# cxm12/TGSR

Measured on AMD Instinct MI355X. Metric: SR images/sec (32->256, batch 16 per GPU, one step in flight), higher is better.
Workload: dtype f32

## Files before the change

### include/tgsr_hip.h

```cpp
#ifndef TGSR_HIP_H
#define TGSR_HIP_H

#include <stdint.h>

#ifdef __cplusplus
extern "C" {
#endif

#define TGSR_OK 0
#define TGSR_EINVAL (-1)
#define TGSR_EUNSUPPORTED (-2)
#define TGSR_ELAUNCH (-3)

#define TGSR_EPI_AFFINE 0
#define TGSR_EPI_AFFINE_GLU 1

#define TGSR_ACT_NONE 0
#define TGSR_ACT_TANH_AXPY 1
#define TGSR_ACT_IDENT_AXPY 2

#define TGSR_ABI_VERSION 2
int tgsr_abi_version(void);
const char* tgsr_last_error(void);

// ... 40 lines not shown
                           float* out, int64_t out_bstride, int epilogue, void* stream);

int tgsr_pack_wino4_wide_weight(const float* w, float* upack, int Cout, int Cin, int glu, void* stream);
int tgsr_pack_wino4_wide_weight_dgrad(const float* w, float* upack, int Cout, int Cin, void* stream);
int tgsr_wino4_wide_stats_nslots(int B, int H, int W, int Cout);
int tgsr_wino4_wide_conv3x3_stats_fwd(const float* x, int64_t x_bstride, int B, int Cin, int H, int W, const float* upack,
                                      int Cout, float* out, int64_t out_bstride, float* stat_partial, void* stream);
int tgsr_wino4_wide_conv3x3_fwd(const float* x, int64_t x_bstride, int B, int Cin, int H, int W, const float* upack, int Cout,
                                const float* scale, const float* shift, const float* residual, int64_t res_bstride,
                                float* out, int64_t out_bstride, int epilogue, void* stream);

int tgsr_conv_to3_set_pipe(int on);

int tgsr_conv_to3_fwd(const float* x, int64_t x_bstride, int B, int Cin, int H, int W, const float* w, int K,
                      int act, const float* addend, float alpha, float* out, void* stream);

int tgsr_word_attention_fwd(const float* h, int64_t h_bstride, const float* words, const float* w_ctx,
                            const uint8_t* mask, int mask_mode, int B, int idf, int cdf, int T, int Q, float* src_ws,
                            float* c_code, int64_t c_bstride, float* attn, void* stream);

int tgsr_word_project_fwd(const float* words, const float* const* w_ctx, int nsets, int B, int idf, int cdf, int T,
                          float* src_out, void* stream);

int tgsr_bilstm_fwd(const int64_t* captions, int width, const int32_t* cap_lens, int B, int Tmax, const float* emb,
                    int ntoken, int ninput, const float* w_ih, const float* w_hh, const float* b_ih,
                    const float* b_hh, int H, float* gates_ws, float* words_emb, float* sent_emb, void* stream);

int tgsr_lstm_gate_table(const float* emb, int ntoken, int ninput, const float* w_ih, const float* b_ih,
                         const float* b_hh, int H, float* table, void* stream);
int tgsr_bilstm_table_fwd(const int64_t* captions, int width, const int32_t* cap_lens, int B, int Tmax,
// ... 271 lines not shown
```

### tgsr_amd/_lib.py

```python
import ctypes
import os
import subprocess

_HERE = os.path.dirname(os.path.abspath(__file__))
LIB_PATH = os.environ.get("TGSR_LIB_PATH") or os.path.join(_HERE, "lib", "libtgsr_hip.so")
ABI_VERSION = 2

OK, EINVAL, EUNSUPPORTED, ELAUNCH = 0, -1, -2, -3
EPI_AFFINE, EPI_AFFINE_GLU = 0, 1
ACT_NONE, ACT_TANH_AXPY, ACT_IDENT_AXPY = 0, 1, 2
DT_BF16, DT_F16 = 1, 2

_vp, _i, _i64, _f, _d = ctypes.c_void_p, ctypes.c_int, ctypes.c_int64, ctypes.c_float, ctypes.c_double

SIGNATURES = {
    "tgsr_abi_version": (_i, []),
    "tgsr_last_error": (ctypes.c_char_p, []),
    "tgsr_packed_weight_elems": (_i64, [_i, _i, _i]),
    "tgsr_pack_conv_weight": (_i, [_vp, _vp, _i, _i, _i, _vp]),
    "tgsr_pack_conv_weight_dgrad": (_i, [_vp, _vp, _i, _i, _i, _vp]),
    "tgsr_bn_fold": (_i, [_vp, _vp, _vp, _vp, _f, _vp, _vp, _i, _vp]),
    "tgsr_conv3x3_fwd": (_i, [_vp, _i64, _i, _i, _i, _i, _vp, _i, _vp, _vp, _vp, _i64, _vp, _i64, _i, _i, _vp]),
    "tgsr_packed_upconv_weight_elems": (_i64, [_i, _i]),
    "tgsr_pack_upconv_weight": (_i, [_vp, _vp, _i, _i, _vp]),
# ... 30 lines not shown
    "tgsr_damsm_words_bwd_ws_elems": (_i64, [_i, _i, _i]),
    "tgsr_damsm_words_bwd": (_i, [_vp, _vp, _vp, _vp, _i, _i, _i, _i, _f, _f, _vp, _vp, _vp, _vp]),
    "tgsr_func_attention_fwd": (_i, [_vp, _vp, _i, _i, _i, _i, _f, _vp, _vp, _vp]),
    "tgsr_conv1x1_fwd": (_i, [_vp, _i, _i, _i, _vp, _vp, _i, _vp, _vp]),
    "tgsr_linear_fwd": (_i, [_vp, _i, _i, _vp, _vp, _i, _vp, _vp]),
    "tgsr_rowdot_fwd": (_i, [_vp, _vp, _vp, _vp, _i, _i, _vp]),
    "tgsr_ca_net_fwd": (_i, [_vp, _vp, _vp, _vp, _i, _i, _i, _vp, _vp, _vp, _vp]),
    "tgsr_rowdot_bwd": (_i, [_vp, _vp, _vp, _vp, _vp, _i, _i, _vp]),
    "tgsr_bn_train_nsplit": (_i, [_i, _i, _i]),
    "tgsr_bn_train_fwd": (_i, [_vp, _i, _i, _i, _vp, _vp, _f, _f, _vp, _vp, _i, _vp, _i64, _vp, _vp, _vp, _vp, _vp, _vp,
                               _i64, _vp, _vp]),
    "tgsr_bn_train_bwd": (_i, [_vp, _vp, _i, _i, _i, _vp, _vp, _vp, _vp, _i, _vp, _vp, _vp, _vp, _vp, _vp]),
    "tgsr_dconv_set_split": (_i, [_i]),
    "tgsr_bn_set_fuse_small": (_i, [_i]),
    "tgsr_conv_to3_set_pipe": (_i, [_i]),
    "tgsr_conv4x4s2_split_form": (_i, [_i, _i, _i, _i, _i, _i]),
    "tgsr_conv3x3_gemm_split_form": (_i, [_i, _i, _i, _i, _i, _i]),
    "tgsr_conv4x4s2_ws_elems": (_i64, [_i, _i, _i, _i, _i, _i]),
    "tgsr_conv4x4s2_fwd": (_i, [_vp, _i, _i, _i, _i, _vp, _i, _i, _vp, _vp, _vp]),
    "tgsr_conv4x4s2_dgrad": (_i, [_vp, _i, _i, _i, _i, _vp, _i, _vp, _vp, _vp]),
    "tgsr_conv4x4s2_wgrad": (_i, [_vp, _vp, _i, _i, _i, _i, _i, _vp, _vp, _vp]),
    "tgsr_conv3x3_gemm_ws_elems": (_i64, [_i, _i, _i, _i, _i, _i]),
    "tgsr_conv3x3_gemm_fwd": (_i, [_vp, _i, _i, _i, _i, _vp, _i, _vp, _vp, _vp]),
    "tgsr_conv3x3_gemm_dgrad": (_i, [_vp, _i, _i, _i, _i, _vp, _i, _vp, _vp, _vp]),
    "tgsr_conv3x3_gemm_wgrad": (_i, [_vp, _vp, _i, _i, _i, _i, _i, _vp, _vp, _vp]),
    "tgsr_leaky_relu": (_i, [_vp, _vp, _vp, _i64, _vp]),
    "tgsr_glu": (_i, [_vp, _vp, _vp, _i64, _i64, _vp]),
    "tgsr_wino_stats_nslots": (_i, [_i, _i, _i, _i]),
    "tgsr_wino_conv3x3_stats_fwd": (_i, [_vp, _i64, _i, _i, _i, _i, _vp, _i, _vp, _i64, _vp, _vp]),
    "tgsr_wino4_stats_nslots": (_i, [_i, _i, _i, _i]),
# ... 135 lines not shown
```

### tgsr_amd/csrc/tgsr_conv_to3.hip

```cpp
#include "tgsr_common.h"

namespace tgsr {

typedef __attribute__((address_space(3))) void* lds_ptr3_t;
typedef const __attribute__((address_space(1))) void* glb_ptr1_t;

__device__ __attribute__((aligned(16))) float g_to3_zero[4] = {0.f, 0.f, 0.f, 0.f};

struct To3Args {
  const float* x;
  int64_t xbs;
  int B, Cin, H, W;
  const float* w;
  const float* addend;
  float alpha;
  float* out;
  int tiles_x, tiles_y;
};

__device__ __forceinline__ float fast_tanh(float v) {
  const float e = __expf(2.f * v);
  return 1.f - 2.f / (e + 1.f);
}

// ... 143 lines not shown
          if (xx + p < a.W) {
            float v = acc[co][p];
            if (ACT == TGSR_ACT_TANH_AXPY) {
              v = fast_tanh(v);
              if (addp) v += a.alpha * addp[o + p];
            }
            outp[o + p] = v;
          }
        }
      }
    }
  }
}


template <int K, int ACT, int TH, int KS>
__global__ __launch_bounds__(16 * TH * KS) void conv_to3_pipe_kernel(To3Args a) {
  constexpr int P = K / 2, CK = 2, TW = 64, NG = 16 * TH, NW = NG / 64, NT = 16 * TH * KS;
  constexpr int TR = TH + K - 1;
  constexpr int PITCH = 72;
  constexpr int STAGE = CK * TR * PITCH;
  constexpr int UK = ((STAGE + 255) / 256 + NW - 1) / NW;
  constexpr int BUF = UK * NW * 256, D = 3;
  constexpr int WPC = (3 * K * K + 3) & ~3;
  static_assert(NG % 64 == 0, "a channel group is a whole number of waves");
  static_assert((KS - 1) * 12 * NG <= KS * D * BUF, "reduction buffer fits the stage buffers");
  __shared__ __attribute__((aligned(16))) float smem_all[KS * D * BUF];
  extern __shared__ __attribute__((aligned(16))) float w_s[];

  const int grp = __builtin_amdgcn_readfirstlane(threadIdx.x / NG);
  const int tid = threadIdx.x - grp * NG, lane = tid & 63;
  const int wave = __builtin_amdgcn_readfirstlane(tid >> 6);
  float* smem = smem_all + grp * D * BUF;
  const int lq = (lane >> 2) & 7;
  const int txi = (lq >> 1) * 4 + (lane & 3), tyi = 4 * wave + 2 * (lane >> 5) + ((0x96 >> lq) & 1);
  int t = xcd_remap(blockIdx.x, gridDim.x);
  const int tx = t % a.tiles_x;
  t /= a.tiles_x;
  const int ty = t % a.tiles_y;
  const int b = t / a.tiles_y;
  const int y0 = ty * TH, x0 = tx * TW;
  const uint32_t HW = (uint32_t)a.H * (uint32_t)a.W;
  const float* xb = a.x + (int64_t)b * a.xbs;

  for (int o = threadIdx.x; o < a.Cin * 3 * K * K; o += NT) {
    const int c = o / (3 * K * K), r = o - c * (3 * K * K);
    const int co = r / (K * K), tp = r - co * (K * K);
    w_s[c * WPC + r] = a.w[((int64_t)co * a.Cin + c) * (K * K) + tp];
  }

  int off[UK];
// ... 13 lines not shown
    for (int k = 0; k < UK; ++k) {
      const int v = off[k];
      const int c = c0 + (v >> 28);
      const bool ok = v >= 0 && c < a.Cin;
      const float* g = ok ? xb + (uint64_t)(uint32_t)c * HW + (uint32_t)(v & 0x0fffffff) : g_to3_zero;
      const unsigned dst = lds0 + (unsigned)(bi * BUF + NW * k * 256) * 4u;
      asm volatile("s_mov_b32 m0, %1\n\ts_nop 0\n\tglobal_load_lds_dwordx4 %0, off" ::"v"(g), "s"(dst) : "memory");
    }
  };

  float acc[3][4];
#pragma unroll
  for (int co = 0; co < 3; ++co)
#pragma unroll
    for (int p = 0; p < 4; ++p) acc[co][p] = 0.f;

  const int nst = (a.Cin + CK - 1) / CK, per = (nst + KS - 1) / KS;
  const int s0 = grp * per, s1 = s0 + per < nst ? s0 + per : nst;
  if (s0 < s1) issue(0, s0 * CK);
  if (s0 + 1 < s1) issue(1, (s0 + 1) * CK);
  __syncthreads();

  int bi = 0;
  for (int i = 0; i < per; ++i) {
    const int st = s0 + i;
    if (st + 1 < s1) asm volatile("s_waitcnt vmcnt(%0)\n\ts_barrier" ::"n"(UK) : "memory");
    else asm volatile("s_waitcnt vmcnt(0)\n\ts_barrier" ::: "memory");
    if (st + 2 < s1) issue(bi >= 1 ? bi - 1 : 2, (st + 2) * CK);
    const float* cur = smem + bi * BUF;
    const int c0 = st * CK;
// ... 34 lines not shown
#pragma unroll
      for (int co = 0; co < 3; ++co)
#pragma unroll
        for (int p = 0; p < 4; ++p) red[((grp - 1) * 12 + co * 4 + p) * NG + tid] = acc[co][p];
    }
    __syncthreads();
    if (grp > 0) return;
#pragma unroll
    for (int g = 1; g < KS; ++g)
#pragma unroll
      for (int co = 0; co < 3; ++co)
#pragma unroll
        for (int p = 0; p < 4; ++p) acc[co][p] += red[((g - 1) * 12 + co * 4 + p) * NG + tid];
  }

  const int y = y0 + tyi, xx = x0 + 4 * txi;
  float* __restrict__ outp = a.out;
  const float* __restrict__ addp = a.addend;
  if (y < a.H && xx < a.W) {
#pragma unroll
    for (int co = 0; co < 3; ++co) {
      const int64_t o = ((int64_t)b * 3 + co) * HW + (int64_t)y * a.W + xx;
      float4 ad = make_float4(0.f, 0.f, 0.f, 0.f);
      if (ACT == TGSR_ACT_TANH_AXPY && addp) ad = *reinterpret_cast<const float4*>(addp + o);
      const float adv[4] = {ad.x, ad.y, ad.z, ad.w};
      float r[4];
#pragma unroll
      for (int p = 0; p < 4; ++p) r[p] = ACT == TGSR_ACT_TANH_AXPY ? fast_tanh(acc[co][p]) + a.alpha * adv[p] : acc[co][p];
      *reinterpret_cast<float4*>(outp + o) = make_float4(r[0], r[1], r[2], r[3]);
    }
  }
}

template <int K, int ACT, int CH, int TRO>
__global__ __launch_bounds__(256) void conv_to3_mfma_kernel(To3Args a) {
  constexpr int RPW = TRO / 4;
  constexpr int NJ = CH / 4;
  constexpr int P = K / 2, ROWS = TRO + K - 1, PITCH = 80;
  constexpr int CS = (ROWS * PITCH) % 64 == 0 ? ROWS * PITCH + 16 : (ROWS * PITCH + 63) / 64 * 64 + 16 - ((ROWS * PITCH) % 64 <= 16 ? 64 : 0);
  static_assert(CS % 64 == 16 && CS >= ROWS * PITCH && CS % 4 == 0, "channel stride");
  constexpr int VP = 84;
  constexpr int SM = CH * CS > 4 * 16 * VP ? CH * CS : 4 * 16 * VP;
  __shared__ __attribute__((aligned(16))) float x_s[SM];
  const int tid = threadIdx.x, lane = tid & 63, wave = tid >> 6, col = lane & 15, kq = lane >> 4;
// ... 94 lines not shown
        if (a.addend) v += a.alpha * a.addend[o];
      }
      a.out[o] = v;
    }
    asm volatile("s_waitcnt lgkmcnt(0)" ::: "memory");
    __builtin_amdgcn_wave_barrier();
  }
}

static int g_to3_pipe = [] {
  const char* e = getenv("TGSR_TO3_PIPE");
  return (e && e[0] == '0') ? 0 : 1;
}();
static bool to3_pipe() { return g_to3_pipe != 0; }

template <int K, int ACT, int TH, int KS>
static int launch_to3_th(To3Args a, hipStream_t s) {
  a.tiles_x = (a.W + 63) / 64;
  a.tiles_y = (a.H + TH - 1) / TH;
  const dim3 grid((unsigned)(a.B * a.tiles_x * a.tiles_y));
  const bool vec4 = (a.W % 4 == 0) && (a.xbs % 4 == 0) && ((reinterpret_cast<uintptr_t>(a.x) & 15) == 0) &&
                    ((reinterpret_cast<uintptr_t>(a.out) & 15) == 0) &&
                    (!a.addend || (reinterpret_cast<uintptr_t>(a.addend) & 15) == 0);
  constexpr int WPC = (3 * K * K + 3) & ~3;
  const size_t wbytes = (size_t)a.Cin * WPC * sizeof(float);
  if (vec4 && wbytes <= 16 * 1024 && to3_pipe())
    hipLaunchKernelGGL((conv_to3_pipe_kernel<K, ACT, TH, KS>), grid, dim3(16 * TH * KS), wbytes, s, a);
  else if (vec4)
    hipLaunchKernelGGL((conv_to3_kernel<K, ACT, true, TH, KS>), grid, dim3(16 * TH * KS), 0, s, a);
  else
    hipLaunchKernelGGL((conv_to3_kernel<K, ACT, false, TH, KS>), grid, dim3(16 * TH * KS), 0, s, a);
  return note_launch(hipGetLastError(), "conv_to3_kernel");
}

template <int K, int ACT>
static int launch_to3(To3Args a, hipStream_t s) {
  auto tiles = [&](int th) { return (int64_t)a.B * ((a.W + 63) / 64) * ((a.H + th - 1) / th); };
  if (K == 5 && a.Cin % 16 == 0 && a.W % 64 == 0 && a.H % 8 == 0 && tiles(8) >= 512 && a.xbs % 4 == 0 &&
      (reinterpret_cast<uintptr_t>(a.x) & 15) == 0) {
    a.tiles_x = a.W / 64;
    a.tiles_y = a.H / 8;
    hipLaunchKernelGGL((conv_to3_mfma_kernel<K, ACT, 8, 8>), dim3((unsigned)(a.B * a.tiles_x * a.tiles_y)), dim3(256), 0, s, a);
    return note_launch(hipGetLastError(), "conv_to3_mfma_kernel");
  }
  if (tiles(16) >= 512) return launch_to3_th<K, ACT, 16, 1>(a, s);
  if (tiles(8) >= 512) return launch_to3_th<K, ACT, 8, 2>(a, s);
  return launch_to3_th<K, ACT, 4, 4>(a, s);
}

}

using namespace tgsr;

extern "C" int tgsr_conv_to3_set_pipe(int on) {
  const int was = g_to3_pipe;
  g_to3_pipe = on ? 1 : 0;
  return was;
}

extern "C" int tgsr_conv_to3_fwd(const float* x, int64_t x_bstride, int B, int Cin, int H, int W, const float* w,
                                 int K, int act, const float* addend, float alpha, float* out, void* stream) {
  if (!x || !w || !out || B < 1 || Cin < 1 || H < 1 || W < 1) return TGSR_EINVAL;
  if (K != 3 && K != 5) return TGSR_EUNSUPPORTED;
  if (act != TGSR_ACT_NONE && act != TGSR_ACT_TANH_AXPY) return TGSR_EINVAL;
  if (act == TGSR_ACT_NONE && addend) return TGSR_EINVAL;
  if ((int64_t)H * W >= (1 << 28) || (int64_t)Cin * H * W >= (1ll << 32)) return TGSR_EUNSUPPORTED;
  To3Args a;
  a.x = x; a.xbs = x_bstride; a.B = B; a.Cin = Cin; a.H = H; a.W = W; a.w = w;
  a.addend = addend; a.alpha = alpha; a.out = out; a.tiles_x = a.tiles_y = 0;
  hipStream_t s = as_stream(stream);
  if (K == 3) return act == TGSR_ACT_NONE ? launch_to3<3, TGSR_ACT_NONE>(a, s) : launch_to3<3, TGSR_ACT_TANH_AXPY>(a, s);
  return act == TGSR_ACT_NONE ? launch_to3<5, TGSR_ACT_NONE>(a, s) : launch_to3<5, TGSR_ACT_TANH_AXPY>(a, s);
}
```

### tgsr_amd/custom_ops.py

```python
from typing import Optional

import torch

from . import lp, ops

_lib = torch.library.Library("tgsr", "DEF")
_T = torch.Tensor


def _refuse_cpu(name):
    def kernel(*args, **kwargs):
        raise ops.TgsrError("torch.ops.tgsr.%s got CPU tensors: tgsr_amd ops run only on HIP tensors; there is no CPU fallback" % name)
    return kernel


def _define(schema, fn, fake=None):
    name = schema.split("(")[0]
    _lib.define(schema)
    _lib.impl(name, fn, "CUDA")
    _lib.impl(name, _refuse_cpu(name), "CPU")
    if fake is not None:
        torch.library.register_fake("tgsr::" + name, fake, lib=_lib)
    return getattr(torch.ops.tgsr, name).default

# ... 388 lines not shown
                    (words.new_empty(len(ws), words.shape[0], ws[0].shape[0], 32), words.new_empty(words.shape[0], ncf),
                     words.new_empty(words.shape[0], ncf),
                     words.new_empty(words.shape[0], words.shape[2], dtype=torch.uint8)))
text_tail_lp = _define("text_tail_lp(Tensor words, Tensor[] w_ctxs, Tensor sent_emb, Tensor ca_w, Tensor ca_b, int ncf, "
                       "Tensor captions, bool bf16) -> (Tensor, Tensor, Tensor, Tensor, Tensor)",
                       lambda words, ws, sent, cw, cb, ncf, cap, bf16:
                       ops.text_tail(words, list(ws), sent, cw, cb, ncf, cap,
                                     lp_dtype=torch.bfloat16 if bf16 else torch.float16),
                       lambda words, ws, sent, cw, cb, ncf, cap, bf16:
                       (words.new_empty(len(ws), words.shape[0], ws[0].shape[0], 32), words.new_empty(words.shape[0], ncf),
                        words.new_empty(words.shape[0], ncf),
                        words.new_empty(words.shape[0], words.shape[2], dtype=torch.uint8),
                        words.new_empty(len(ws) * words.shape[0] * 4096 + 4 * words.shape[0], dtype=torch.uint8)))
axpy_images = _define("axpy_images(Tensor[] ts, Tensor[] ss, float alpha) -> Tensor[]",
                      lambda ts, ss, alpha: ops.axpy_images(list(ts), list(ss), alpha), lambda ts, ss, alpha: [torch.empty_like(t) for t in ts])
gconv_pack = _define("gconv_pack(Tensor w, Tensor? scale, bool dgrad) -> Tensor", lambda w, sc, dg: ops.gconv_pack(w, sc, dg),
                     lambda w, sc, dg: w.new_empty((w.shape[1], w.shape[0] * w.shape[2] * w.shape[3]) if dg else
                                                   (w.shape[0], w.shape[1] * w.shape[2] * w.shape[3])))
gconv = _define("gconv(bool dgrad, Tensor A, Tensor S, int s_coff, int s_ch, Tensor(a!) out, int o_coff, int kh, int kw, int stride, "
                "int padh, int padw, Tensor? bias, bool relu, bool accumulate, Tensor(b!)? ws, Tensor? mask) -> ()",
                lambda dg, A, S, sc, sch, out, oc, kh, kw, st, ph, pw, bias, relu, acc, ws, mask:
                ops.gconv(dg, A, S, sc, sch, out, oc, kh, kw, st, ph, pw, bias, relu, acc, ws, mask), lambda *a: None)
gconv_stats = _define("gconv_stats(Tensor A, Tensor S, int s_coff, int s_ch, Tensor(a!) out, int o_coff, int kh, int kw, int stride, "
                      "int padh, int padw, Tensor(b!)? ws, Tensor(c!) stat_partial) -> ()",
                      lambda A, S, sc, sch, out, oc, kh, kw, st, ph, pw, ws, part:
                      (ops.gconv_stats(A, S, sc, sch, out, oc, kh, kw, st, ph, pw, ws, part), None)[1], lambda *a: None)
bn_train_relu_slice_from_stats = _define(
    "bn_train_relu_slice_from_stats(Tensor(a!) y, int coff, Tensor gamma, Tensor beta, float eps, float momentum, "
    "Tensor(b!)? running_mean, Tensor(c!)? running_var, Tensor(d!)? num_batches_tracked, Tensor stat_partial, int slot_px, "
    "Tensor(e!) stats) -> ()",
# ... 162 lines not shown
```

### tgsr_amd/model.py

```python
import torch
import torch.nn as nn
import torch.nn.functional as F
from torch.autograd import Variable

from . import custom_ops as C
from . import ops
from .miscc.config import cfg
from .util import (CA_NET, CNN_ENCODER, D_GET_LOGITS, GET_IMAGE_G, GET_IMAGE_G_noAct, GLU, INIT_STAGE_GImgup, NEXT_STAGE_G,
                   RNN_ENCODER, ResBlock, Block3x3_leakRelu, Block3x3_relu, _ConvBnGlu, _ResidualNoSum, conv1x1, conv3x3,
                   conv5x5, downBlock, encode_image_by_16times, upBlock)

__all__ = ["G_SR_NET_low", "G_SR_NET_low_stage1", "NetG_highweight", "RNN_ENCODER", "CNN_ENCODER", "CA_NET",
           "INIT_STAGE_GImgup", "NEXT_STAGE_G", "GET_IMAGE_G", "GET_IMAGE_G_noAct", "ResBlock", "GLU", "upBlock",
           "Block3x3_relu", "conv1x1", "conv3x3", "conv5x5", "Variable", "cfg", "torch", "nn", "F",
           "D_NET64", "D_NET128", "D_NET256", "D_GET_LOGITS", "downBlock", "Block3x3_leakRelu"]


class G_SR_NET_low_stage1(nn.Module):

    def __init__(self, *args, **kwargs):
        super(G_SR_NET_low_stage1, self).__init__()
        raise NotImplementedError("G_SR_NET_low_stage1 is dead code in the reference (stage1=False, "
                                  "trainer_objective.py:56); tgsr_amd builds G_SR_NET_low")

# ... 4 lines not shown
        super(G_SR_NET_low, self).__init__()
        ngf = cfg.GAN.GF_DIM
        nef = cfg.TEXT.EMBEDDING_DIM
        ncf = cfg.GAN.CONDITION_DIM
        self.ca_net = CA_NET()
        self.h_net1 = INIT_STAGE_GImgup(ngf, ncf, nef)
        self.h_net2 = NEXT_STAGE_G(ngf, nef, ncf)
        self.h_net3 = NEXT_STAGE_G(ngf, nef, ncf)
        self.img_net1 = GET_IMAGE_G_noAct(ngf)
        self.img_net2 = GET_IMAGE_G_noAct(ngf)
        self.img_net3 = GET_IMAGE_G_noAct(ngf)

    def attention_modules(self):
        return [self.h_net1.att, self.h_net2.att, self.h_net3.att]

    def forward(self, LR, sent_emb, word_embs, mask, outmiddle=False, ca=None, proj=None):
        fake_imgs, att_maps = [], []
        c_code, mu, logvar = self.ca_net(sent_emb) if ca is None else ca
        srcs = [None, None, None]
        if proj is not None:
            srcs = proj
        elif not self.training:
            srcs = C.word_project(word_embs, [a.conv_context.weight.detach() for a in self.attention_modules()])
        h_code1, att0 = self.h_net1(None, LR, word_embs, mask, wide_out=True, src=srcs[0])
        fake_imgs.append(self.img_net1(h_code1))
        att_maps.append(att0)
        h_code2, att1 = self.h_net2(h_code1, None, word_embs, mask, wide_out=True, src=srcs[1])
        fake_imgs.append(self.img_net2(h_code2))
        att_maps.append(att1)
        h_code3, att2 = self.h_net3(h_code2, None, word_embs, mask, src=srcs[2])
        fake_imgs.append(self.img_net3(h_code3))
        att_maps.append(att2)
        if outmiddle:
            return fake_imgs, att_maps, mu, logvar, [h_code1, h_code2, h_code3]
        return fake_imgs, att_maps, mu, logvar


class NetG_highweight(nn.Module):

    MAP_SIZES = (64, 128, 256)

    def __init__(self, weightmap=False, low='lr-lrblur', useAct=True):
        super(NetG_highweight, self).__init__()
        ngf = cfg.GAN.GF_DIM
        self.low = low
        self.useAct = bool(useAct)
        self.residual = nn.Sequential(*[ResBlock(channel_num=32) for _ in range(6)])
# ... 45 lines not shown
        out8 = self.upscale8x(self.residual48(out4))
        return out2, out4, out8

    def heads(self, feats, SRb):
        return [self._head(f, sr, k) for k, (f, sr) in enumerate(zip(feats, SRb))]

    def tanh_heads(self, feats):
        w = self.conv_output[0].weight.detach()
        return [C.conv_to3(f, w, self.useAct, None, self._a) for f in feats]

    def finish_heads(self, ts, SRb):
        if self.weightmap:
            return [C.axpy_map(t, s.contiguous(), a.detach()) for t, s, a in zip(ts, SRb, self.maps())]
        return list(C.axpy_images(list(ts), [s.contiguous() for s in SRb[:len(ts)]], self._a))

    def forward(self, LR, SRb, LRb):
        ims = self.heads(self.trunk(LR, LRb), SRb[:3])
        a, one = self._const(LR)
        if self.weightmap:
            return ims, self.a3, one
        return ims, a, one


class _D_NET(nn.Module):

    def __init__(self, extra_down, b_jcu=True):
        super().__init__()
        ndf, nef = cfg.GAN.DF_DIM, cfg.TEXT.EMBEDDING_DIM
        self.img_code_s16 = encode_image_by_16times(ndf)
        ch = ndf * 8
# ... 37 lines not shown
```

### tgsr_amd/ops.py

```python
import collections
import ctypes
import functools
import os
from typing import Optional, Tuple

import torch

from . import _lib
from ._lib import TgsrError, check

BN_EPS = 1e-5

profile = None


def _ev():
    e = torch.cuda.Event(enable_timing=True)
    e.record()
    return e


_raw_stream = getattr(torch._C, "_cuda_getCurrentRawStream", None)


# ... 384 lines not shown
        if tuple(addend.shape) != (B, 3, H, W):
            raise TgsrError("conv_to3: addend shape %s" % (tuple(addend.shape),))
    out = torch.empty(B, 3, H, W, dtype=torch.float32, device=x.device)
    e0 = _ev() if profile is not None else None
    rc = _lib.lib().tgsr_conv_to3_fwd(_p(x), xbs, B, Cin, H, W, _p(w), int(w.shape[2]),
                                      _lib.ACT_TANH_AXPY if tanh_axpy else _lib.ACT_NONE, _p(addend), float(alpha),
                                      _p(out), _stream())
    check(rc, "tgsr_conv_to3_fwd")
    if profile is not None:
        K = int(w.shape[2])
        nbytes = 4 * (B * Cin * H * W + B * 3 * H * W * (2 if addend is not None else 1))
        profile.append(("conv_to3_kernel", 2.0 * B * H * W * 3 * Cin * K * K, nbytes, e0, _ev()))
    return out


_MASK_CACHE = [None, None, None]


def _mask_u8(mask: torch.Tensor) -> torch.Tensor:
    if mask.dtype == torch.uint8 and mask.is_contiguous():
        return mask
    if mask.dtype == torch.bool and mask.is_contiguous():
        return mask.view(torch.uint8)
    key = (mask.data_ptr(), mask._version, tuple(mask.shape), mask.dtype)
    if _MASK_CACHE[0] != key or _MASK_CACHE[1] is not mask:
        _MASK_CACHE[0], _MASK_CACHE[1], _MASK_CACHE[2] = key, mask, mask.to(torch.uint8).contiguous()
    return _MASK_CACHE[2]


def word_project(words: torch.Tensor, w_ctxs) -> list:
# ... 334 lines not shown
    b = None if bias is None else _f32(bias.detach(), "bias").contiguous()
    if CONV1X1_GCONV and K % 16 == 0 and K >= 256:
        xt = x.t().contiguous().view(1, K, B, 1)
        img = torch.empty(1, w2.shape[0], B, 1, dtype=torch.float32, device=x.device)
        need = gconv_ws_elems(1, w2.shape[0], B, 1, K)
        ws = torch.empty(need, dtype=torch.float32, device=x.device) if need else None
        gconv(False, w2, xt, 0, K, img, 0, 1, 1, 1, 0, 0, b, False, False, ws, None)
        return img.view(w2.shape[0], B).t().contiguous()
    out = torch.empty(B, w2.shape[0], dtype=torch.float32, device=x.device)
    check(_lib.lib().tgsr_linear_fwd(_p(x), B, K, _p(w2), _p(b), w2.shape[0], _p(out), _stream()), "tgsr_linear_fwd")
    return out


def conv_to3_set_pipe(on: bool) -> bool:
    return bool(_lib.lib().tgsr_conv_to3_set_pipe(1 if on else 0))


def bn_set_fuse_small(on: bool) -> bool:
    return bool(_lib.lib().tgsr_bn_set_fuse_small(1 if on else 0))


def bn_train_fwd(raw: torch.Tensor, gamma: torch.Tensor, beta: torch.Tensor, eps: float, momentum: float,
                 running_mean: Optional[torch.Tensor], running_var: Optional[torch.Tensor], act: int = 0,
                 residual: Optional[torch.Tensor] = None, nbt: Optional[torch.Tensor] = None,
                 out: Optional[torch.Tensor] = None, stats: Optional[torch.Tensor] = None,
                 stat_partial: Optional[torch.Tensor] = None):
    _need_hip(raw, gamma, beta, running_mean, running_var, residual, nbt, out, stats, stat_partial)
    L = _lib.lib()
    B, C, Ho, Wo = raw.shape
    HW, dev = Ho * Wo, raw.device
# ... 862 lines not shown
```

### tgsr_amd/trainer.py

```python
import os

import numpy as np

import torch

from .miscc.config import cfg
from . import custom_ops as C
from . import ops
from .model import RNN_ENCODER


def sort_by_caption_length(captions, cap_lens, *per_sample):
    lens, idx = torch.sort(cap_lens, 0, True)
    return (captions[idx], lens) + tuple(t[idx] for t in per_sample) + (idx,)


def caption_mask(captions, num_words):
    return (captions[:, :num_words] if captions.size(1) > num_words else captions) == 0


def to_uint8(img):
    if img.is_cuda:
        from . import custom_ops as C
        return C.to_uint8(img.detach()).cpu().numpy()
    a = img.detach().cpu().numpy()
    return np.round(np.maximum(0, np.minimum(255, (a + 1.0) * 127.5))).astype(np.uint8)


GH_AFTER_TEXT = int(os.environ.get("TGSR_GH_AFTER_TEXT", "-1"))
SPLIT_HEADS = os.environ.get("TGSR_SPLIT_HEADS", "1") != "0"


def crop_words(out, num_words):
    T = int(num_words)
    if out["words_emb"].size(2) == T:
        return out
    res = dict(out)
    res["words_emb"] = out["words_emb"][:, :, :T]
    res["mask"] = out["mask"][:, :T]
    res["att"] = [a[:, :T] for a in out["att"]]
    return res


class _ProjWithPack(list):

# ... 156 lines not shown
        if pack is not None:
            proj = _ProjWithPack(proj, pack)
        return proj, (None, mu, logvar), m8.view(torch.bool)

    def _forward(self, captions, cap_lens, LR, LRb):
        hidden = None
        if self._lp is not None:
            ex = self._lp
            ex.refresh()
            bufs = ex._buffers(LR.shape[0], LR.shape[2], LR.shape[3], LR.device)
            trunk = lambda: ex.high_trunk(bufs, LR, LRb)
            low = lambda sent, words, mask, ca, proj: ex.low(bufs, LR, sent, words, mask, ca=ca, proj=proj,
                                                             defer_heads=True)
            heads = ex.high_heads
        elif SPLIT_HEADS and not self.netGH.training:
            trunk = lambda: self.netGH.tanh_heads(self.netGH.trunk(LR, LRb))
            low = lambda sent, words, mask, ca, proj: self.netGL(LR, sent, words, mask, ca=ca, proj=proj)
            heads = self.netGH.finish_heads
        else:
            trunk = lambda: self.netGH.trunk(LR, LRb)
            low = lambda sent, words, mask, ca, proj: self.netGL(LR, sent, words, mask, ca=ca, proj=proj)
            heads = self.netGH.heads
        feats = side = None

        def fork_trunk(start=None):
            nonlocal feats, side
            main_ = torch.cuda.current_stream(LR.device)
            if self._side is None:
                self._side = {}
            side = self._side.get(main_.cuda_stream)
            if side is None:
                side = self._side[main_.cuda_stream] = distinct_streams(1, LR.device, avoid=[main_.cuda_stream])[0]
            if start is not None:
# ... 153 lines not shown
```

Measured before the change: 12180.

## Fold final to-RGB conv and residual axpy heads into one launch

Adds a variant of the pipelined 3-channel output conv kernel. It computes the last scale's image and writes both it and its residual-blended fine image. Extra trailing blocks in the same grid run the float4 axpy for the two earlier scales. The inference path in the trainer defers the last low-branch head and calls this combined op instead of a separate to-RGB conv plus an axpy launch, saving a launch and one round trip of the last image through memory. In exchange it adds a restricted path: pipe form only, no weightmap, no grad.

```diff
diff --git a/include/tgsr_hip.h b/include/tgsr_hip.h
--- a/include/tgsr_hip.h
+++ b/include/tgsr_hip.h
@@ -78,6 +78,10 @@
 
 int tgsr_conv_to3_fwd(const float* x, int64_t x_bstride, int B, int Cin, int H, int W, const float* w, int K,
                       int act, const float* addend, float alpha, float* out, void* stream);
+
+int tgsr_conv_to3_finish_fwd(const float* x, int64_t x_bstride, int B, int Cin, int H, int W, const float* w, int K, float* out,
+                             int n, float* const* fine, const float* const* t, const float* const* s, const int64_t* numel,
+                             float alpha, void* stream);
 
 int tgsr_word_attention_fwd(const float* h, int64_t h_bstride, const float* words, const float* w_ctx,
                             const uint8_t* mask, int mask_mode, int B, int idf, int cdf, int T, int Q, float* src_ws,
diff --git a/tgsr_amd/_lib.py b/tgsr_amd/_lib.py
--- a/tgsr_amd/_lib.py
+++ b/tgsr_amd/_lib.py
@@ -68,6 +68,7 @@
     "tgsr_dconv_set_split": (_i, [_i]),
     "tgsr_bn_set_fuse_small": (_i, [_i]),
     "tgsr_conv_to3_set_pipe": (_i, [_i]),
+    "tgsr_conv_to3_finish_fwd": (_i, [_vp, _i64, _i, _i, _i, _i, _vp, _i, _vp, _i, _vp, _vp, _vp, _vp, _f, _vp]),
     "tgsr_conv4x4s2_split_form": (_i, [_i, _i, _i, _i, _i, _i]),
     "tgsr_conv3x3_gemm_split_form": (_i, [_i, _i, _i, _i, _i, _i]),
     "tgsr_conv4x4s2_ws_elems": (_i64, [_i, _i, _i, _i, _i, _i]),
diff --git a/tgsr_amd/csrc/tgsr_conv_to3.hip b/tgsr_amd/csrc/tgsr_conv_to3.hip
--- a/tgsr_amd/csrc/tgsr_conv_to3.hip
+++ b/tgsr_amd/csrc/tgsr_conv_to3.hip
@@ -181,9 +181,20 @@
 }
 
 
-template <int K, int ACT, int TH, int KS>
-__global__ __launch_bounds__(16 * TH * KS) void conv_to3_pipe_kernel(To3Args a) {
-  constexpr int P = K / 2, CK = 2, TW = 64, NG = 16 * TH, NW = NG / 64, NT = 16 * TH * KS;
+struct To3Fin {
+  const float* t_last;
+  float* fine_last;
+  const float* t[2];
+  const float* s[2];
+  float* fine[2];
+  uint32_t n4[2];
+  float alpha;
+  int conv_blocks;
+};
+
+template <int K, int ACT, int TH, int KS, bool FIN>
+__global__ __launch_bounds__(16 * TH * KS) void conv_to3_pipe_kernel(To3Args a, To3Fin f) {
+  constexpr int P = K / 2, CK = 2, TW = 64, NG = 16 * TH, NW = NG / 64, NT = NG * KS;
   constexpr int TR = TH + K - 1;
   constexpr int PITCH = 72;
   constexpr int STAGE = CK * TR * PITCH;
@@ -192,8 +203,31 @@
   constexpr int WPC = (3 * K * K + 3) & ~3;
   static_assert(NG % 64 == 0, "a channel group is a whole number of waves");
   static_assert((KS - 1) * 12 * NG <= KS * D * BUF, "reduction buffer fits the stage buffers");
+  static_assert(!FIN || ACT == TGSR_ACT_NONE, "the closing launch has no activation");
   __shared__ __attribute__((aligned(16))) float smem_all[KS * D * BUF];
   extern __shared__ __attribute__((aligned(16))) float w_s[];
+
+  const int nconv = FIN ? f.conv_blocks : (int)gridDim.x;
+  if (FIN && (int)blockIdx.x >= nconv) {
+    const uint32_t e = blockIdx.x - nconv, ne = gridDim.x - nconv;
+    const float al = f.alpha;
+#pragma unroll
+    for (int k = 0; k < 2; ++k) {
+      const float4* __restrict__ t4 = reinterpret_cast<const float4*>(f.t[k]);
+      const float4* __restrict__ s4 = reinterpret_cast<const float4*>(f.s[k]);
+      float4* __restrict__ o4 = reinterpret_cast<float4*>(f.fine[k]);
+      for (uint32_t i = e * NT + threadIdx.x; i < f.n4[k]; i += ne * NT) {
+        const float4 tv = t4[i], sv = s4[i];
+        float4 r;
+        r.x = fmaf(al, sv.x, tv.x);
+        r.y = fmaf(al, sv.y, tv.y);
+        r.z = fmaf(al, sv.z, tv.z);
+        r.w = fmaf(al, sv.w, tv.w);
+        o4[i] = r;
+      }
+    }
+    return;
+  }
 
   const int grp = __builtin_amdgcn_readfirstlane(threadIdx.x / NG);
   const int tid = threadIdx.x - grp * NG, lane = tid & 63;
@@ -201,7 +235,7 @@
   float* smem = smem_all + grp * D * BUF;
   const int lq = (lane >> 2) & 7;
   const int txi = (lq >> 1) * 4 + (lane & 3), tyi = 4 * wave + 2 * (lane >> 5) + ((0x96 >> lq) & 1);
-  int t = xcd_remap(blockIdx.x, gridDim.x);
+  int t = xcd_remap(blockIdx.x, nconv);
   const int tx = t % a.tiles_x;
   t /= a.tiles_x;
   const int ty = t % a.tiles_y;
@@ -245,6 +279,15 @@
   for (int co = 0; co < 3; ++co)
 #pragma unroll
     for (int p = 0; p < 4; ++p) acc[co][p] = 0.f;
+
+  const int y = y0 + tyi, xx = x0 + 4 * txi;
+  float* __restrict__ outp = a.out;
+  const float* __restrict__ addp = a.addend;
+  float4 tl[3] = {};
+  if (FIN && grp == 0 && y < a.H && xx < a.W) {
+#pragma unroll
+    for (int co = 0; co < 3; ++co) tl[co] = *reinterpret_cast<const float4*>(f.t_last + ((int64_t)b * 3 + co) * HW + (int64_t)y * a.W + xx);
+  }
 
   const int nst = (a.Cin + CK - 1) / CK, per = (nst + KS - 1) / KS;
   const int s0 = grp * per, s1 = s0 + per < nst ? s0 + per : nst;
@@ -309,20 +352,21 @@
         for (int p = 0; p < 4; ++p) acc[co][p] += red[((g - 1) * 12 + co * 4 + p) * NG + tid];
   }
 
-  const int y = y0 + tyi, xx = x0 + 4 * txi;
-  float* __restrict__ outp = a.out;
-  const float* __restrict__ addp = a.addend;
   if (y < a.H && xx < a.W) {
 #pragma unroll
     for (int co = 0; co < 3; ++co) {
       const int64_t o = ((int64_t)b * 3 + co) * HW + (int64_t)y * a.W + xx;
       float4 ad = make_float4(0.f, 0.f, 0.f, 0.f);
       if (ACT == TGSR_ACT_TANH_AXPY && addp) ad = *reinterpret_cast<const float4*>(addp + o);
+      if (FIN) ad = tl[co];
       const float adv[4] = {ad.x, ad.y, ad.z, ad.w};
-      float r[4];
-#pragma unroll
-      for (int p = 0; p < 4; ++p) r[p] = ACT == TGSR_ACT_TANH_AXPY ? fast_tanh(acc[co][p]) + a.alpha * adv[p] : acc[co][p];
-      *reinterpret_cast<float4*>(outp + o) = make_float4(r[0], r[1], r[2], r[3]);
+      float v[4];
+#pragma unroll
+      for (int p = 0; p < 4; ++p) v[p] = ACT == TGSR_ACT_TANH_AXPY ? fast_tanh(acc[co][p]) + a.alpha * adv[p] : acc[co][p];
+      *reinterpret_cast<float4*>(outp + o) = make_float4(v[0], v[1], v[2], v[3]);
+      if (FIN)
+        *reinterpret_cast<float4*>(f.fine_last + o) = make_float4(fmaf(f.alpha, v[0], adv[0]), fmaf(f.alpha, v[1], adv[1]),
+                                                                  fmaf(f.alpha, v[2], adv[2]), fmaf(f.alpha, v[3], adv[3]));
     }
   }
 }
@@ -447,38 +491,60 @@
 }();
 static bool to3_pipe() { return g_to3_pipe != 0; }
 
-template <int K, int ACT, int TH, int KS>
-static int launch_to3_th(To3Args a, hipStream_t s) {
-  a.tiles_x = (a.W + 63) / 64;
-  a.tiles_y = (a.H + TH - 1) / TH;
-  const dim3 grid((unsigned)(a.B * a.tiles_x * a.tiles_y));
+enum To3Form { TO3_MFMA, TO3_PIPE, TO3_VEC4, TO3_SCALAR };
+
+static int64_t to3_tiles(const To3Args& a, int th) { return (int64_t)a.B * ((a.W + 63) / 64) * ((a.H + th - 1) / th); }
+static int to3_th(const To3Args& a) { return to3_tiles(a, 16) >= 512 ? 16 : to3_tiles(a, 8) >= 512 ? 8 : 4; }
+
+static To3Form to3_form(const To3Args& a, int K) {
+  if (K == 5 && a.Cin % 16 == 0 && a.W % 64 == 0 && a.H % 8 == 0 && to3_tiles(a, 8) >= 512 && a.xbs % 4 == 0 &&
+      (reinterpret_cast<uintptr_t>(a.x) & 15) == 0)
+    return TO3_MFMA;
   const bool vec4 = (a.W % 4 == 0) && (a.xbs % 4 == 0) && ((reinterpret_cast<uintptr_t>(a.x) & 15) == 0) &&
                     ((reinterpret_cast<uintptr_t>(a.out) & 15) == 0) &&
                     (!a.addend || (reinterpret_cast<uintptr_t>(a.addend) & 15) == 0);
-  constexpr int WPC = (3 * K * K + 3) & ~3;
-  const size_t wbytes = (size_t)a.Cin * WPC * sizeof(float);
-  if (vec4 && wbytes <= 16 * 1024 && to3_pipe())
-    hipLaunchKernelGGL((conv_to3_pipe_kernel<K, ACT, TH, KS>), grid, dim3(16 * TH * KS), wbytes, s, a);
-  else if (vec4)
-    hipLaunchKernelGGL((conv_to3_kernel<K, ACT, true, TH, KS>), grid, dim3(16 * TH * KS), 0, s, a);
-  else
-    hipLaunchKernelGGL((conv_to3_kernel<K, ACT, false, TH, KS>), grid, dim3(16 * TH * KS), 0, s, a);
+  const size_t wbytes = (size_t)a.Cin * ((3 * K * K + 3) & ~3) * sizeof(float);
+  if (vec4 && wbytes <= 16 * 1024 && to3_pipe()) return TO3_PIPE;
+  return vec4 ? TO3_VEC4 : TO3_SCALAR;
+}
+
+template <int K, int ACT, int TH, int KS>
+static int launch_to3_th(To3Args a, To3Form form, const To3Fin* fin, int extra_blocks, hipStream_t s) {
+  a.tiles_x = (a.W + 63) / 64;
+  a.tiles_y = (a.H + TH - 1) / TH;
+  const unsigned tiles = (unsigned)(a.B * a.tiles_x * a.tiles_y);
+  const size_t wbytes = (size_t)a.Cin * ((3 * K * K + 3) & ~3) * sizeof(float);
+  if (form == TO3_PIPE && fin) {
+    if constexpr (ACT == TGSR_ACT_NONE) {
+      To3Fin f = *fin;
+      f.conv_blocks = (int)tiles;
+      hipLaunchKernelGGL((conv_to3_pipe_kernel<K, ACT, TH, KS, true>), dim3(tiles + (unsigned)extra_blocks), dim3(16 * TH * KS),
+                         wbytes, s, a, f);
+    }
+  } else if (form == TO3_PIPE) {
+    hipLaunchKernelGGL((conv_to3_pipe_kernel<K, ACT, TH, KS, false>), dim3(tiles), dim3(16 * TH * KS), wbytes, s, a, To3Fin{});
+  } else if (form == TO3_VEC4) {
+    hipLaunchKernelGGL((conv_to3_kernel<K, ACT, true, TH, KS>), dim3(tiles), dim3(16 * TH * KS), 0, s, a);
+  } else {
+    hipLaunchKernelGGL((conv_to3_kernel<K, ACT, false, TH, KS>), dim3(tiles), dim3(16 * TH * KS), 0, s, a);
+  }
   return note_launch(hipGetLastError(), "conv_to3_kernel");
 }
 
 template <int K, int ACT>
-static int launch_to3(To3Args a, hipStream_t s) {
-  auto tiles = [&](int th) { return (int64_t)a.B * ((a.W + 63) / 64) * ((a.H + th - 1) / th); };
-  if (K == 5 && a.Cin % 16 == 0 && a.W % 64 == 0 && a.H % 8 == 0 && tiles(8) >= 512 && a.xbs % 4 == 0 &&
-      (reinterpret_cast<uintptr_t>(a.x) & 15) == 0) {
+static int launch_to3(To3Args a, const To3Fin* fin, int extra_blocks, hipStream_t s) {
+  const To3Form form = to3_form(a, K);
+  if (form == TO3_MFMA) {
     a.tiles_x = a.W / 64;
     a.tiles_y = a.H / 8;
     hipLaunchKernelGGL((conv_to3_mfma_kernel<K, ACT, 8, 8>), dim3((unsigned)(a.B * a.tiles_x * a.tiles_y)), dim3(256), 0, s, a);
     return note_launch(hipGetLastError(), "conv_to3_mfma_kernel");
   }
-  if (tiles(16) >= 512) return launch_to3_th<K, ACT, 16, 1>(a, s);
-  if (tiles(8) >= 512) return launch_to3_th<K, ACT, 8, 2>(a, s);
-  return launch_to3_th<K, ACT, 4, 4>(a, s);
+  switch (to3_th(a)) {
+    case 16: return launch_to3_th<K, ACT, 16, 1>(a, form, fin, extra_blocks, s);
+    case 8: return launch_to3_th<K, ACT, 8, 2>(a, form, fin, extra_blocks, s);
+    default: return launch_to3_th<K, ACT, 4, 4>(a, form, fin, extra_blocks, s);
+  }
 }
 
 }
@@ -491,17 +557,53 @@
   return was;
 }
 
+static int to3_args(To3Args& a, const float* x, int64_t x_bstride, int B, int Cin, int H, int W, const float* w, int K, float* out) {
+  if (!x || !w || !out || B < 1 || Cin < 1 || H < 1 || W < 1) return TGSR_EINVAL;
+  if (K != 3 && K != 5) return TGSR_EUNSUPPORTED;
+  if ((int64_t)H * W >= (1 << 28) || (int64_t)Cin * H * W >= (1ll << 32)) return TGSR_EUNSUPPORTED;
+  a.x = x; a.xbs = x_bstride; a.B = B; a.Cin = Cin; a.H = H; a.W = W; a.w = w;
+  a.addend = nullptr; a.alpha = 0.f; a.out = out; a.tiles_x = a.tiles_y = 0;
+  return TGSR_OK;
+}
+
 extern "C" int tgsr_conv_to3_fwd(const float* x, int64_t x_bstride, int B, int Cin, int H, int W, const float* w,
                                  int K, int act, const float* addend, float alpha, float* out, void* stream) {
-  if (!x || !w || !out || B < 1 || Cin < 1 || H < 1 || W < 1) return TGSR_EINVAL;
-  if (K != 3 && K != 5) return TGSR_EUNSUPPORTED;
+  To3Args a;
+  if (const int rc = to3_args(a, x, x_bstride, B, Cin, H, W, w, K, out)) return rc;
   if (act != TGSR_ACT_NONE && act != TGSR_ACT_TANH_AXPY) return TGSR_EINVAL;
   if (act == TGSR_ACT_NONE && addend) return TGSR_EINVAL;
-  if ((int64_t)H * W >= (1 << 28) || (int64_t)Cin * H * W >= (1ll << 32)) return TGSR_EUNSUPPORTED;
+  a.addend = addend; a.alpha = alpha;
+  hipStream_t s = as_stream(stream);
+  if (K == 3) return act == TGSR_ACT_NONE ? launch_to3<3, TGSR_ACT_NONE>(a, nullptr, 0, s) : launch_to3<3, TGSR_ACT_TANH_AXPY>(a, nullptr, 0, s);
+  return act == TGSR_ACT_NONE ? launch_to3<5, TGSR_ACT_NONE>(a, nullptr, 0, s) : launch_to3<5, TGSR_ACT_TANH_AXPY>(a, nullptr, 0, s);
+}
+
+extern "C" int tgsr_conv_to3_finish_fwd(const float* x, int64_t x_bstride, int B, int Cin, int H, int W, const float* w, int K,
+                                        float* out, int n, float* const* fine, const float* const* t, const float* const* s,
+                                        const int64_t* numel, float alpha, void* stream) {
   To3Args a;
-  a.x = x; a.xbs = x_bstride; a.B = B; a.Cin = Cin; a.H = H; a.W = W; a.w = w;
-  a.addend = addend; a.alpha = alpha; a.out = out; a.tiles_x = a.tiles_y = 0;
-  hipStream_t s = as_stream(stream);
-  if (K == 3) return act == TGSR_ACT_NONE ? launch_to3<3, TGSR_ACT_NONE>(a, s) : launch_to3<3, TGSR_ACT_TANH_AXPY>(a, s);
-  return act == TGSR_ACT_NONE ? launch_to3<5, TGSR_ACT_NONE>(a, s) : launch_to3<5, TGSR_ACT_TANH_AXPY>(a, s);
-}
+  if (const int rc = to3_args(a, x, x_bstride, B, Cin, H, W, w, K, out)) return rc;
+  if (n < 1 || !fine || !t || !s || !numel) return TGSR_EINVAL;
+  if (n > 3) return TGSR_EUNSUPPORTED;
+  To3Fin f{};
+  uint32_t most = 0;
+  for (int i = 0; i < n; ++i) {
+    const bool last = i == n - 1;
+    if (!fine[i] || !t[i] || (!last && !s[i]) || numel[i] < 1) return TGSR_EINVAL;
+    if (last && numel[i] != (int64_t)B * 3 * H * W) return TGSR_EINVAL;
+    if ((numel[i] & 3) || numel[i] > 0x7fffffff ||
+        ((reinterpret_cast<uintptr_t>(fine[i]) | reinterpret_cast<uintptr_t>(t[i]) | (last ? 0 : reinterpret_cast<uintptr_t>(s[i]))) & 15))
+      return TGSR_EUNSUPPORTED;
+    if (last) {
+      f.t_last = t[i]; f.fine_last = fine[i];
+    } else {
+      f.t[i] = t[i]; f.s[i] = s[i]; f.fine[i] = fine[i]; f.n4[i] = (uint32_t)(numel[i] >> 2);
+      most = f.n4[i] > most ? f.n4[i] : most;
+    }
+  }
+  f.alpha = alpha;
+  if (to3_form(a, K) != TO3_PIPE) return TGSR_EUNSUPPORTED;
+  const int extra = (int)((most + 255) / 256 < 256 ? (most + 255) / 256 : 256);
+  hipStream_t st = as_stream(stream);
+  return K == 3 ? launch_to3<3, TGSR_ACT_NONE>(a, &f, extra, st) : launch_to3<5, TGSR_ACT_NONE>(a, &f, extra, st);
+}
diff --git a/tgsr_amd/custom_ops.py b/tgsr_amd/custom_ops.py
--- a/tgsr_amd/custom_ops.py
+++ b/tgsr_amd/custom_ops.py
@@ -426,6 +426,10 @@
                         words.new_empty(len(ws) * words.shape[0] * 4096 + 4 * words.shape[0], dtype=torch.uint8)))
 axpy_images = _define("axpy_images(Tensor[] ts, Tensor[] ss, float alpha) -> Tensor[]",
                       lambda ts, ss, alpha: ops.axpy_images(list(ts), list(ss), alpha), lambda ts, ss, alpha: [torch.empty_like(t) for t in ts])
+conv_to3_finish = _define("conv_to3_finish(Tensor x, Tensor w, Tensor[] ts, Tensor[] ss, float alpha) -> (Tensor, Tensor[])",
+                          lambda x, w, ts, ss, alpha: ops.conv_to3_finish(x, w, list(ts), list(ss), alpha),
+                          lambda x, w, ts, ss, alpha: (x.new_empty(x.shape[0], 3, x.shape[2], x.shape[3]),
+                                                       [torch.empty_like(t) for t in ts]))
 gconv_pack = _define("gconv_pack(Tensor w, Tensor? scale, bool dgrad) -> Tensor", lambda w, sc, dg: ops.gconv_pack(w, sc, dg),
                      lambda w, sc, dg: w.new_empty((w.shape[1], w.shape[0] * w.shape[2] * w.shape[3]) if dg else
                                                    (w.shape[0], w.shape[1] * w.shape[2] * w.shape[3])))
diff --git a/tgsr_amd/model.py b/tgsr_amd/model.py
--- a/tgsr_amd/model.py
+++ b/tgsr_amd/model.py
@@ -42,7 +42,7 @@
     def attention_modules(self):
         return [self.h_net1.att, self.h_net2.att, self.h_net3.att]
 
-    def forward(self, LR, sent_emb, word_embs, mask, outmiddle=False, ca=None, proj=None):
+    def forward(self, LR, sent_emb, word_embs, mask, outmiddle=False, ca=None, proj=None, defer_last_head=False):
         fake_imgs, att_maps = [], []
         c_code, mu, logvar = self.ca_net(sent_emb) if ca is None else ca
         srcs = [None, None, None]
@@ -57,8 +57,12 @@
         fake_imgs.append(self.img_net2(h_code2))
         att_maps.append(att1)
         h_code3, att2 = self.h_net3(h_code2, None, word_embs, mask, src=srcs[2])
+        att_maps.append(att2)
+        if defer_last_head:
+            if outmiddle:
+                raise ValueError("G_SR_NET_low: outmiddle returns every image, defer_last_head leaves the last one out")
+            return fake_imgs, att_maps, mu, logvar, (h_code3, self.img_net3.img[0].weight)
         fake_imgs.append(self.img_net3(h_code3))
-        att_maps.append(att2)
         if outmiddle:
             return fake_imgs, att_maps, mu, logvar, [h_code1, h_code2, h_code3]
         return fake_imgs, att_maps, mu, logvar
@@ -134,6 +138,14 @@
             return [C.axpy_map(t, s.contiguous(), a.detach()) for t, s, a in zip(ts, SRb, self.maps())]
         return list(C.axpy_images(list(ts), [s.contiguous() for s in SRb[:len(ts)]], self._a))
 
+    def finish_heads_with_last(self, ts, SRb, last):
+        if self.weightmap:
+            raise ValueError("NetG_highweight(weightmap=True) has no folded closing launch; use finish_heads")
+        h_code, w = last
+        img, fine = C.conv_to3_finish(h_code, w.detach(), list(ts), [s.contiguous() for s in SRb], self._a)
+        SRb.append(img)
+        return list(fine)
+
     def forward(self, LR, SRb, LRb):
         ims = self.heads(self.trunk(LR, LRb), SRb[:3])
         a, one = self._const(LR)
diff --git a/tgsr_amd/ops.py b/tgsr_amd/ops.py
--- a/tgsr_amd/ops.py
+++ b/tgsr_amd/ops.py
@@ -422,6 +422,42 @@
     return out
 
 
+def conv_to3_finish(x: torch.Tensor, w: torch.Tensor, ts, ss, alpha: float):
+    import ctypes
+    ts, ss = list(ts), list(ss)
+    n = len(ts)
+    if n < 1 or n > 3 or len(ss) != n - 1:
+        raise TgsrError("conv_to3_finish: %d / %d images (1..3 scales, one low-frequency image fewer)" % (n, len(ss)))
+    _need_hip(x, w, *ts, *ss)
+    x, xbs = _nchw_bstride(_f32(x, "x"), "x")
+    w = _f32(w.detach(), "w").contiguous()
+    B, Cin, H, W = x.shape
+    if w.shape[0] != 3 or w.shape[1] != Cin or w.shape[2] != w.shape[3]:
+        raise TgsrError("conv_to3_finish: weight shape %s" % (tuple(w.shape),))
+    ts = [_f32(t, "t").contiguous() for t in ts]
+    ss = [_f32(s_, "s").contiguous() for s_ in ss]
+    if tuple(ts[-1].shape) != (B, 3, H, W):
+        raise TgsrError("conv_to3_finish: last scale %s against a %s head" % (tuple(ts[-1].shape), (B, 3, H, W)))
+    for t, s_ in zip(ts, ss):
+        if t.shape != s_.shape:
+            raise TgsrError("conv_to3_finish: %s + alpha * %s" % (tuple(t.shape), tuple(s_.shape)))
+    img = torch.empty(B, 3, H, W, dtype=torch.float32, device=x.device)
+    fine = [torch.empty_like(t) for t in ts]
+    tp = (ctypes.c_void_p * n)(*[t.data_ptr() for t in ts])
+    sp = (ctypes.c_void_p * n)(*([s_.data_ptr() for s_ in ss] + [None]))
+    fp = (ctypes.c_void_p * n)(*[o.data_ptr() for o in fine])
+    ne = (ctypes.c_int64 * n)(*[t.numel() for t in ts])
+    e0 = _ev() if profile is not None else None
+    rc = _lib.lib().tgsr_conv_to3_finish_fwd(_p(x), xbs, B, Cin, H, W, _p(w), int(w.shape[2]), _p(img), n, fp, tp, sp, ne,
+                                             float(alpha), _stream())
+    check(rc, "tgsr_conv_to3_finish_fwd")
+    if profile is not None:
+        K = int(w.shape[2])
+        nbytes = 4 * (B * Cin * H * W + B * 3 * H * W) + 4 * sum(3 * t.numel() for t in ts) - 4 * ts[-1].numel()
+        profile.append(("conv_to3_kernel", 2.0 * B * H * W * 3 * Cin * K * K, nbytes, e0, _ev()))
+    return img, fine
+
+
 _MASK_CACHE = [None, None, None]
 
 
@@ -786,6 +822,13 @@
 
 def conv_to3_set_pipe(on: bool) -> bool:
     return bool(_lib.lib().tgsr_conv_to3_set_pipe(1 if on else 0))
+
+
+def conv_to3_pipe() -> bool:
+    L = _lib.lib()
+    was = L.tgsr_conv_to3_set_pipe(1)
+    L.tgsr_conv_to3_set_pipe(was)
+    return bool(was)
 
 
 def bn_set_fuse_small(on: bool) -> bool:
diff --git a/tgsr_amd/trainer.py b/tgsr_amd/trainer.py
--- a/tgsr_amd/trainer.py
+++ b/tgsr_amd/trainer.py
@@ -29,6 +29,7 @@
 
 GH_AFTER_TEXT = int(os.environ.get("TGSR_GH_AFTER_TEXT", "-1"))
 SPLIT_HEADS = os.environ.get("TGSR_SPLIT_HEADS", "1") != "0"
+FOLD_FINISH = os.environ.get("TGSR_FOLD_FINISH", "1") != "0"
 
 
 def crop_words(out, num_words):
@@ -215,9 +216,13 @@
                                                              defer_heads=True)
             heads = ex.high_heads
         elif SPLIT_HEADS and not self.netGH.training:
+            from . import model as _m8
+            fold = (FOLD_FINISH and LR.is_cuda and isinstance(self.netGL, _m8.G_SR_NET_low) and not self.netGL.training
+                    and not self.netGH.weightmap and not torch.is_grad_enabled() and LR.shape[3] % 4 == 0 and ops.conv_to3_pipe())
             trunk = lambda: self.netGH.tanh_heads(self.netGH.trunk(LR, LRb))
-            low = lambda sent, words, mask, ca, proj: self.netGL(LR, sent, words, mask, ca=ca, proj=proj)
-            heads = self.netGH.finish_heads
+            low = lambda sent, words, mask, ca, proj: self.netGL(LR, sent, words, mask, ca=ca, proj=proj,
+                                                                 **({"defer_last_head": True} if fold else {}))
+            heads = self.netGH.finish_heads_with_last if fold else self.netGH.finish_heads
         else:
             trunk = lambda: self.netGH.trunk(LR, LRb)
             low = lambda sent, words, mask, ca, proj: self.netGL(LR, sent, words, mask, ca=ca, proj=proj)
```

Result: faster. 12460 (median of 6 runs) (+2.3%).
